# PSeitz/veloci

Measured on AMD Instinct MI355X. Metric: queries/sec, 3-term AND on 100M-doc index (p50 latency and HBM fraction alongside), higher is better.
Workload: dtype u32 doc ids + f16->f32 scores

## Files before the change

veloci_amd/csrc/capi.cpp:

```cpp
#include <chrono>
#include <thread>
#include <cstdio>
#include <cstdlib>
#include <cstring>

#include "../../include/veloci_amd.h"
#include <functional>
#include <future>

#include <dlfcn.h>
#include <unistd.h>

#include "engine.hpp"
#include "text.hpp"

using namespace vq;
using vqreq::Request;
using vqreq::VelociError;

namespace {
thread_local std::string g_err;

int fail(int code, const std::string& msg) {
    g_err = msg;
// ... 238 lines not shown
template <class F>
int debug_run(const vq_index* index, F body) {
    try {
        bool fits = true;
        vq::debug_prepass(*index->idx, [&](Workspace& ws, hipStream_t st) { fits = body(ws, st); });
        g_err.clear();
        return fits ? 0 : -2;
    } catch (const std::exception& e) {
        g_err = e.what();
        return -1;
    }
}
}

extern "C" {

const char* vq_last_error(void) { return g_err.c_str(); }
const char* vq_version(void) { return "veloci_amd 0.5 (gfx950)"; }
uint32_t vq_debug_div100_mismatches(void) { return vq::debug_div100_mismatches(); }
uint32_t vq_debug_probe_occupancy(uint32_t shape, uint32_t nd, uint32_t na, uint32_t arr_slot, uint32_t cand_cap, uint32_t* lds_bytes) {
    const size_t lds = vq::scan_probe_lds_bytes(cand_cap, nd, na, arr_slot);
    if (lds_bytes) *lds_bytes = uint32_t(lds);
    return vq::debug_probe_occupancy(shape, lds);
}
uint64_t vq_index_speculative_reruns(const vq_index* index) { return index ? index->idx->or_reruns.load() : 0; }
void vq_index_suggest_topn_probes(const vq_index* index, uint64_t* topn_probes, uint64_t* records_copied_back) {
    if (topn_probes) *topn_probes = index ? index->idx->suggest_topn_probes.load() : 0;
    if (records_copied_back) *records_copied_back = index ? index->idx->suggest_records_back.load() : 0;
}
int vq_debug_dict_topn(const uint32_t* terms, const uint32_t* classes, uint32_t n, uint32_t top_n, uint32_t* out_terms, uint32_t* out_classes, uint32_t* out_n) {
    if ((n && (!terms || !classes)) || !out_terms || !out_classes || !out_n || top_n == 0 || top_n > vq::kTopnMax) return -2;
    for (uint32_t i = 0; i < n; ++i)
        if (classes[i] >= vq::kTopnClasses) return -2;
    uint16_t ord[vq::kTopnClasses];
    vq::topn_class_ords(ord);
    return vq::debug_dict_topn(terms, classes, n, top_n, ord, out_terms, out_classes, out_n);
}
void vq_index_highlight_rank_counts(const vq_index* index, uint64_t* device_parts, uint64_t* snippets_built) {
    if (device_parts) *device_parts = index ? index->idx->highlight_device_parts.load() : 0;
    if (snippets_built) *snippets_built = index ? index->idx->highlight_snippets_built.load() : 0;
}
int vq_debug_text_rank(const uint64_t* row_off, const uint32_t* row_vals, const uint32_t* row_score_bits, uint32_t num_rows, uint32_t num_texts, uint32_t top_n,
                       uint32_t* out_texts, uint32_t* out_score_bits, uint32_t* out_n, uint32_t* out_touched) {
    if (!row_off || (num_rows && !row_score_bits) || !out_texts || !out_score_bits || !out_n || !out_touched) return -2;
    if (top_n == 0 || top_n > vq::kTextRankMaxTop || num_texts == 0 || uint64_t(num_texts) * 4 > vq::kTextRankBudget || row_off[0] != 0) return -2;
    for (uint32_t r = 0; r < num_rows; ++r) {
// ... 1389 lines not shown
```

veloci_amd/csrc/compile.cpp:

```cpp
#include <algorithm>
#include <cmath>
#include <cstdlib>
#include <cstring>
#include <regex>
#include <set>

#include "engine.hpp"
#include "text.hpp"

namespace vq {
std::atomic<uint64_t> g_compile_ns[16];

using namespace vqreq;

namespace {

bool ends_with(const std::string& s, const char* suf) {
    size_t n = std::strlen(suf);
    return s.size() >= n && std::memcmp(s.data() + s.size() - n, suf, n) == 0;
}

[[noreturn]] void unsupported(const std::string& what) {
    throw VelociError(ERR_UNSUPPORTED, "unsupported on the MI355X query path: " + what);
}
// ... 660 lines not shown
                }
                cq.algorithmic_bytes += 6ull * done->input_postings + 8ull * done->len;
                info.glen = done->global_len;
                info.len_known = !req.filtered() && idx.can_sum_over_shards();
            }
            op.list_count = uint16_t(count);
            push_op(ops, op, sp);
            info.emitted = true;
            return info;
        }
        uint32_t with_entries = 0;
        for (auto& e : entries) {
            const PostingStore& ps = *e.ps;
            if (ps.global_len[e.tid]) ++with_entries;
            if (ps.len[e.tid] == 0) continue;
            HList h;
            h.d_docs = ps.docs.as<uint32_t>() + ps.start[e.tid];
            h.d_scores = ps.scores.as<uint16_t>() + ps.start[e.tid];
            h.len = ps.len[e.tid];
            h.global_len = ps.global_len[e.tid];
            h.flags = LIST_HAS_SCORES;
            h.term_score = e.score;
            h.max_raw = ps.max_raw[e.tid];
            if (!ps.bm_start.empty() && ps.bm_start[e.tid] >= 0) {
                h.flags |= LIST_BITMAP;
                h.d_bitmap = ps.bitmaps.as<uint32_t>() + ps.bm_start[e.tid];
                h.d_rank_dir = ps.rank_dir.as<uint32_t>() + ps.rd_start[e.tid];
            }
            if (!ps.td_start.empty() && ps.td_start[e.tid] >= 0) h.d_tile_dir = ps.tile_dir.as<uint32_t>() + ps.td_start[e.tid];
            if (!ps.pk_start.empty() && ps.pk_start[e.tid] >= 0) {
                h.d_cov32 = ps.cov32.as<uint32_t>() + uint64_t(ps.pk_start[e.tid]) * 8;
                h.d_gdir = ps.gdir.as<uint32_t>() + ps.gd_start[e.tid];
                if (ps.ak_start[e.tid] >= 0) h.d_arr16 = ps.arr16.as<uint16_t>() + uint64_t(ps.ak_start[e.tid]) * 8;
                h.tile_most = ps.tile_most[e.tid];
            }
            uint32_t li = add_list(h);
            info.cover.push_back(li);
            info.cover_len += h.len;
            cq.algorithmic_bytes += 6ull * h.len;
            ++count;
        }
        op.list_count = uint16_t(count);
        info.len_known = with_entries <= 1 && !req.filtered();
        info.glen = 0;
        for (auto& e : entries) info.glen += e.ps->global_len[e.tid];
        push_op(ops, op, sp);
// ... 2132 lines not shown
```

veloci_amd/csrc/device_types.hpp:

```cpp
#pragma once
#include <hip/hip_runtime.h>
#include <stdint.h>

namespace vq {

constexpr int kBlock = 64;
constexpr int kCandCap = 2048;
constexpr int kMaxTopK = 1024;
constexpr int kStackDepth = 16;
constexpr int kMaxChildren = 16;
constexpr int kMaxLists = 64;
constexpr int kMaxOps = 160;
constexpr int kMaxSkipWhen = 4;
constexpr uint32_t kTileDirShift = 14;
constexpr uint32_t kProbeTileShift = 15;
constexpr uint32_t kRankShift = 9;

enum ListFlags : uint32_t {
    LIST_HAS_SCORES = 1u,
    LIST_COVER = 2u,
    LIST_BITMAP = 4u,
    LIST_F32 = 8u,
};

struct DList {
    const uint32_t* docs;
    const uint16_t* scores;
    uint32_t len;
    uint32_t flags;
    float term_score;
    uint16_t max_raw;
    uint16_t pad;
    const uint32_t* bitmap;
    const uint32_t* rank_dir;
    const uint32_t* tile_dir;
};

enum OpKind : uint8_t { OP_LEAF = 0, OP_AND = 1, OP_OR = 2, OP_BOOST1N = 3, OP_LEAFMAX = 4 };

struct DOp {
    uint8_t kind;
    uint8_t nchild;
    uint8_t nslots;
    uint8_t pad;
    uint16_t list_begin;
    uint16_t list_count;
    uint8_t child_slot[kMaxChildren];
    uint8_t and_order[kMaxChildren];
};

enum PresKind : uint8_t { PRES_AND = 0, PRES_OR = 1, PRES_ZERO = 2, PRES_COUNT = 3 };
constexpr uint16_t kSlotTemp = 0x8000;
constexpr uint16_t kSlotRoot = 0xFFFF;
struct DPresOp {
    uint8_t kind;
// ... 166 lines not shown
```

veloci_amd/csrc/engine.hpp:

```cpp
#pragma once
#include <hip/hip_runtime.h>

#include <atomic>
#include <cmath>
#include <chrono>
#include <cstdint>
#include <map>
#include <limits>
#include <memory>
#include <thread>
#include <functional>
#include <condition_variable>
#include <mutex>
#include <string>
#include <unordered_map>
#include <vector>

#include "device_types.hpp"
#include "kernels.hpp"
#include "request.hpp"
#include "hostpool.hpp"
#include "regex_dfa.hpp"

namespace vq {
// ... 268 lines not shown
    uint32_t len = 0;
    uint32_t total = 0;
    bool ascending = true;
    bool several = false;
    bool done = false;
};
using Boost1nTable = std::map<std::string, Boost1nJob>;
constexpr int kStatusNeedsUnion = -1;
constexpr int kStatusNeedsCounts = -2;
constexpr int kStatusNeedsRanges = -3;

struct QueryCounts {
    bool has_filter = false;
    uint64_t filter_count = 0;
    std::map<uint32_t, std::pair<uint64_t, uint64_t>> nodes;
};

struct PostingStore {
    uint32_t num_tokens = 0;
    std::vector<uint64_t> start;
    std::vector<uint32_t> len;
    std::vector<uint64_t> global_len;
    std::vector<uint16_t> max_raw;
    DevBuf docs;
    DevBuf scores;
    uint64_t total_padded = 0;
    std::vector<int64_t> bm_start;
    std::vector<int64_t> rd_start;
    DevBuf bitmaps;
    DevBuf rank_dir;
    std::vector<int64_t> td_start;
    DevBuf tile_dir;
    std::vector<int64_t> pk_start;
    std::vector<int64_t> ak_start;
    std::vector<int64_t> gd_start;
    std::vector<uint32_t> tile_most;
    DevBuf cov32, arr16, gdir;
};

struct KVStore {
    uint32_t key_base = 0, num_keys = 0;
    std::vector<uint64_t> host_off;
    std::vector<uint32_t> host_values;
    bool list_rows = false;
    bool rows_sorted_unique = true;
    bool rows_equal_postings = false;
// ... 193 lines not shown
};

std::unique_ptr<Index> build_index(const IndexBuilder& b, int device);

struct DocSet {
    uint64_t index_uid = 0;
    uint32_t num_anchors = 0, doc_lo = 0, doc_hi = 0;
    uint64_t len = 0;
    uint32_t local_len = 0;
    uint64_t bitmap_words = 0, rank_entries = 0, tile_entries = 0;
    DevBuf docs, bitmap, rank_dir, tile_dir;
    uint64_t device_bytes = 0;
    float ms_mark = -1.0f, ms_count_scan = -1.0f, ms_expand = -1.0f;
};
std::shared_ptr<const DocSet> make_docset(const Index& idx, const uint32_t* ids, uint64_t n, bool on_device);

struct HList {
    const uint32_t* d_docs = nullptr;
    const uint16_t* d_scores = nullptr;
    uint32_t len = 0;
    uint32_t flags = 0;
    float term_score = 0.f;
    uint16_t max_raw = 0x7C00;
    float max_value = std::numeric_limits<float>::infinity();
    uint64_t global_len = 0;
    const uint32_t* d_bitmap = nullptr;
    const uint32_t* d_rank_dir = nullptr;
    const uint32_t* d_tile_dir = nullptr;
    const uint32_t* d_cov32 = nullptr;
    const uint16_t* d_arr16 = nullptr;
    const uint32_t* d_gdir = nullptr;
    uint32_t tile_most = 0;
    int inline_idx = -1;
    int inline_val_idx = -1;
};

struct FacetOut {
    std::string field;
    std::string dict_path;
    uint32_t top = 10;
    uint32_t num_values = 0;
    uint32_t host_top = 0;
};

struct ExplainRec {
    enum Kind : uint8_t { Boost, MaxTokenToTextId, TermToAnchor, LevenshteinScore, OrSumOverDistinctTerms } kind = Boost;
// ... 156 lines not shown
```

veloci_amd/csrc/exec.cpp:

```cpp
#include <algorithm>
#include <cstdio>
#include <cstdlib>
#include <cstring>
#include <thread>

#include "engine.hpp"

#include "text.hpp"

namespace vq {

using namespace vqreq;

void DevBuf::ensure(size_t n) {
    if (n <= bytes) return;
    size_t want = std::max(n, bytes + bytes / 2);
    alloc(want);
}
PinnedBuf::~PinnedBuf() {
    if (p) (void)hipHostFree(p);
}
void PinnedBuf::ensure(size_t n) {
    if (n <= bytes) return;
    if (p) (void)hipHostFree(p);
// ... 121 lines not shown
    h.top_k = cq.top_k;
    h.tile_words = cq.tile_words;
    h.n_spans = cq.n_spans;
    h.keys_base = keys_base;
    h.doc_lo = idx.doc_lo;
    h.doc_hi = idx.doc_hi;
    h.part_keys_off = part_keys_off;
    h.stat_off = stat_off;
    h.blob_bytes = uint32_t(off);
    if (!dst) return off;

    std::memcpy(dst, &h, sizeof h);
    if (h.off_pool) std::memset(dst + h.off_pool, 0, sizeof(DPool) + 8 * size_t(cq.top_k));
    DList* dl = reinterpret_cast<DList*>(dst + h.off_lists);
    for (size_t i = 0; i < cq.lists.size(); ++i) {
        const HList& l = cq.lists[i];
        DList d{};
        d.docs = l.inline_idx >= 0 ? reinterpret_cast<const uint32_t*>(dev + inline_off[l.inline_idx]) : l.d_docs;
        d.scores = l.inline_val_idx >= 0 ? reinterpret_cast<const uint16_t*>(dev + inline_val_off[l.inline_val_idx]) : l.d_scores;
        d.len = l.len;
        d.flags = l.flags;
        d.term_score = l.term_score;
        d.max_raw = l.max_raw;
        d.bitmap = l.d_bitmap;
        d.rank_dir = l.d_rank_dir;
        d.tile_dir = l.d_tile_dir;
        dl[i] = d;
    }
    if (!cq.ops.empty()) std::memcpy(dst + h.off_ops, cq.ops.data(), cq.ops.size() * sizeof(DOp));
    if (!cq.fops.empty()) std::memcpy(dst + h.off_fops, cq.fops.data(), cq.fops.size() * sizeof(DOp));
    if (!cq.groups.empty()) std::memcpy(dst + h.off_groups, cq.groups.data(), cq.groups.size() * sizeof(DGroup));
    if (!cq.tboosts.empty()) std::memcpy(dst + h.off_tboost, cq.tboosts.data(), cq.tboosts.size() * sizeof(DTermBoost));
    if (!cq.cols.empty()) std::memcpy(dst + h.off_col, cq.cols.data(), cq.cols.size() * sizeof(DColBoost));
    if (!cq.locf.empty()) std::memcpy(dst + h.off_locf, cq.locf.data(), cq.locf.size() * sizeof(DLocField));
    if (!cq.loc_idx.empty()) std::memcpy(dst + h.off_loc_idx, cq.loc_idx.data(), cq.loc_idx.size() * sizeof(uint16_t));
    if (sf_rich(cq.simple_flags)) std::memcpy(dst + h.off_simple2, &cq.simple2, sizeof(DSimple2));
    if (sf_wide(cq.simple_flags)) std::memcpy(dst + h.off_simple2, &cq.wide, sizeof(DWide));
    if (sf_probe(cq.simple_flags) || sf_union_packed(cq.simple_flags)) std::memcpy(dst + h.off_simple2, &cq.probe, sizeof(DProbe));
    if (!cq.pres.empty()) std::memcpy(dst + h.off_pres, cq.pres.data(), cq.pres.size() * sizeof(DPresOp));
    if (!cq.pres_in.empty()) std::memcpy(dst + h.off_pres_in, cq.pres_in.data(), cq.pres_in.size() * sizeof(uint16_t));
    DFacet* df = reinterpret_cast<DFacet*>(dst + h.off_facets);
    for (size_t i = 0; i < cq.facets.size(); ++i) {
        DFacet f = cq.facets[i];
        f.hist_off = i < hist_off.size() ? hist_off[i] : 0u;
        f.out_off = i < fac_out_off.size() ? fac_out_off[i] : 0u;
        df[i] = f;
// ... 2431 lines not shown
```

veloci_amd/csrc/index.cpp:

```cpp
#include <algorithm>
#include <atomic>
#include <chrono>
#include <cstring>
#include <exception>
#include <mutex>
#include <thread>
#include <sys/mman.h>

#include "engine.hpp"
#include "text.hpp"

namespace vq {

const char* const TOKENS_TO_TEXT_ID = ".tokens_to_text_id";
const char* const TO_ANCHOR_ID_SCORE = ".to_anchor_id_score";
const char* const PHRASE_PAIR_TO_ANCHOR = ".phrase_pair_to_anchor";
const char* const VALUE_ID_TO_PARENT = ".value_id_to_parent";
const char* const PARENT_TO_VALUE_ID = ".parent_to_value_id";
const char* const TEXT_ID_TO_ANCHOR = ".text_id_to_anchor";
const char* const ANCHOR_TO_TEXT_ID = ".anchor_to_text_id";
const char* const BOOST_VALID_TO_VALUE = ".boost_valid_to_value";
const char* const TOKEN_VALUES = ".token_values";
const char* const VALUE_ID_TO_ANCHOR = ".value_id_to_anchor";
const char* const TEXTINDEX = ".textindex";

static bool ends_with(const std::string& s, const char* suf) {
    size_t n = std::strlen(suf);
    return s.size() >= n && std::memcmp(s.data() + s.size() - n, suf, n) == 0;
}

void DevBuf::alloc(size_t n) {
    release();
    bytes = n;
    if (n == 0) return;
    VQ_HIP(hipMalloc(&p, n));
// ... 273 lines not shown
            }
            std::vector<uint32_t> tdir(tiled.size() * (tiles + 1));
            parallel_for(tiled.size(), nthreads, [&](size_t j) {
                const uint32_t t = tiled[j];
                const uint32_t* d = docs.data() + ps.start[t];
                uint32_t* out = tdir.data() + j * (tiles + 1);
                uint32_t i = 0;
                for (uint64_t k = 0; k <= tiles; ++k) {
                    const uint64_t bound = uint64_t(idx->bitmap_base) + (k << kTileDirShift);
                    while (i < ps.len[t] && d[i] < bound) ++i;
                    out[k] = i;
                }
            });
            if (!tdir.empty()) {
                ps.tile_dir.alloc(tdir.size() * 4 + 16);
                ps.tile_dir.upload(tdir.data(), tdir.size() * 4);
                idx->device_bytes += ps.tile_dir.bytes;
            }
        }
        ps.pk_start.assign(ps.num_tokens, -1);
        ps.ak_start.assign(ps.num_tokens, -1);
        ps.gd_start.assign(ps.num_tokens, -1);
        ps.tile_most.assign(ps.num_tokens, 0);
        {
            const uint64_t ptiles = (idx->bitmap_words >> (kProbeTileShift - 5)) + 2;
            uint64_t cov_gran = 0, arr_gran = 0;
            std::vector<uint32_t> gd(tiled.size() * (ptiles + 1));
            std::vector<uint64_t> gran_of(tiled.size());
            std::vector<uint32_t> most_of(tiled.size());
            parallel_for(tiled.size(), nthreads, [&](size_t j) {
                const uint32_t t = tiled[j];
                const uint32_t* d = docs.data() + ps.start[t];
                uint32_t* g = gd.data() + j * (ptiles + 1);
                uint64_t gran = 0;
                uint32_t i = 0, most = 0;
                for (uint64_t k = 0; k <= ptiles; ++k) {
                    g[k] = uint32_t(gran);
                    const uint64_t thi = uint64_t(idx->bitmap_base) + ((k + 1) << kProbeTileShift);
                    const uint32_t i0 = i;
                    while (i < ps.len[t] && d[i] < thi) ++i;
                    const uint32_t n8 = (i - i0 + 7u) / 8u;
                    most = std::max(most, n8);
                    gran += n8;
                }
                gran_of[j] = gran;
                most_of[j] = most;
// ... 3 lines not shown
                ps.gd_start[t] = int64_t(j * (ptiles + 1));
                if (gran_of[j] >= (1ull << 28)) throw VelociError(vqreq::ERR_INVALID_ARGUMENT, "posting list too long for its tile-packed image");
                ps.pk_start[t] = int64_t(cov_gran);
                ps.tile_most[t] = most_of[j];
                cov_gran += gran_of[j];
                if (most_of[j] <= 256) {
                    ps.ak_start[t] = int64_t(arr_gran);
                    arr_gran += gran_of[j];
                }
            }
            if (cov_gran) {
                ps.cov32.alloc(cov_gran * 32 + 4096);
                ps.arr16.alloc(arr_gran * 16 + 4096);
                ps.gdir.alloc(gd.size() * 4 + 16);
                ps.gdir.upload(gd.data(), gd.size() * 4);
                idx->device_bytes += ps.cov32.bytes + ps.arr16.bytes + ps.gdir.bytes;
                uninit_vector<uint32_t> cov(cov_gran * 8);
                uninit_vector<uint16_t> arr(arr_gran * 8);
                parallel_for(tiled.size(), nthreads, [&](size_t j) {
                    const uint32_t t = tiled[j];
                    const bool as_array = ps.ak_start[t] >= 0;
                    const uint32_t* d = docs.data() + ps.start[t];
                    const uint16_t* sc = scores.data() + ps.start[t];
                    uint32_t* c = cov.data() + uint64_t(ps.pk_start[t]) * 8;
                    uint16_t* a = as_array ? arr.data() + uint64_t(ps.ak_start[t]) * 8 : nullptr;
                    uint64_t w = 0;
                    uint32_t i = 0;
                    for (uint64_t k = 0; k <= ptiles; ++k) {
                        const uint64_t tlo = uint64_t(idx->bitmap_base) + (k << kProbeTileShift), thi = tlo + (1u << kProbeTileShift);
                        for (; i < ps.len[t] && d[i] < thi; ++i, ++w) {
                            const uint32_t rel = uint32_t(d[i] - tlo);
                            c[w] = rel << 16 | sc[i];
                            if (a) a[w] = uint16_t(rel);
                        }
                        for (; w % 8; ++w) {
                            c[w] = 0xFFFFFFFFu;
                            if (a) a[w] = 0xFFFFu;
                        }
                    }
                });
                upload(ps.cov32, cov.data(), cov.size() * 4);
                upload(ps.arr16, arr.data(), arr.size() * 2);
            }
        }
        ps.docs.alloc(docs.size() * 4 + 16);
        upload(ps.docs, docs.data(), docs.size() * 4);
        ps.scores.alloc(scores.size() * 2 + 16);
        upload(ps.scores, scores.data(), scores.size() * 2);
        idx->device_bytes += ps.docs.bytes + ps.scores.bytes;
        idx->postings.emplace(path, std::move(ps));
    }

    for (auto& [path, k] : b.kv) {
        KVStore s;
        s.key_base = k.key_base;
        s.num_keys = uint32_t(k.offsets.size() - 1);
// ... 204 lines not shown
```

veloci_amd/csrc/probe_common.hpp:

```cpp
#pragma once
#include <hip/hip_runtime.h>
#include <hip/hip_fp16.h>

#include "device_types.hpp"
#include "kernel_common.hpp"

namespace vq {

__device__ __forceinline__ unsigned long long wballot(bool p) { return __builtin_amdgcn_ballot_w64(p); }

constexpr uint32_t kPT = 1u << kProbeTileShift;
constexpr uint32_t kPTW = kPT / 32;
constexpr uint32_t kPNV = kPTW / 256;
constexpr uint32_t kPRk = kPT >> kRankShift;
constexpr uint32_t kShCts = 0, kShTs = 1, kShVmax = 4, kShSrc = 7, kShPrunable = 11, kShScores = 12;

__device__ __forceinline__ void probe_lds_fence() { asm volatile("s_waitcnt lgkmcnt(0)" ::: "memory"); }

template <uint32_t ND>
struct ProbeShape {
    float cts, ts[ND], vmax[ND];
    uint32_t src[ND + 1];
    bool prunable;
};
template <uint32_t ND>
__device__ __forceinline__ ProbeShape<ND> probe_shape(const uint32_t* sh) {
    ProbeShape<ND> S;
    S.cts = __uint_as_float(sh[kShCts]);
#pragma unroll
    for (uint32_t i = 0; i < ND; ++i) {
        S.ts[i] = __uint_as_float(sh[kShTs + i]);
        S.vmax[i] = __uint_as_float(sh[kShVmax + i]);
    }
#pragma unroll
    for (uint32_t j = 0; j <= ND; ++j) S.src[j] = sh[kShSrc + j];
    S.prunable = sh[kShPrunable] != 0u;
    return S;
}
// ... 13 lines not shown
}

template <uint32_t ND>
__device__ __forceinline__ float probe_or_sum(const ProbeShape<ND>& S, float vc, const float (&vd)[ND], uint32_t mask) {
    float sum = 0.0f, nd = 0.0f;
#pragma unroll
    for (uint32_t j = 0; j <= ND; ++j) {
        float v = vc;
        bool present = true;
#pragma unroll
        for (uint32_t i = 0; i < ND; ++i)
            if (S.src[j] == 1u + i) {
                v = vd[i];
                present = ((mask >> i) & 1u) != 0u;
            }
        const float m = present ? fmaxf(0.0f, v) : 0.0f;
        if (m >= 0.00001f) nd += 1.0f;
        sum += m;
    }
    return sum * nd * nd;
}

template <uint32_t ND>
__device__ __forceinline__ uint32_t probe_raw_min(const uint32_t* sh, float thr_f, const uint32_t lane, const uint32_t or_mask = 0xFFFFFFFFu) {
    const ProbeShape<ND> S = probe_shape<ND>(sh);
    if (!S.prunable) return 0u;
    uint32_t lo = 0u, hi = 0x7C00u;
    while (hi > lo) {
        const uint32_t step = (hi - lo + 63u) >> 6;
        const uint32_t p = lo + lane * step;
        bool dead = false;
        if (p < hi) {
            const float vc = posting_value_fast(S.cts, (uint16_t)p);
            dead = (or_mask == 0xFFFFFFFFu ? probe_sum<ND>(S, vc, S.vmax) : probe_or_sum<ND>(S, vc, S.vmax, or_mask)) < thr_f;
        }
        const uint32_t c = (uint32_t)__popcll(wballot(dead));
        if (c == 0u) hi = lo;
        else {
            const uint32_t last = lo + (c - 1u) * step;
            const uint32_t nhi = last + step;
            lo = last + 1u;
            hi = nhi < hi ? nhi : hi;
        }
    }
    return lo;
}

template <bool WG>
__device__ void probe_pool_merge(const CandState& cs, uint32_t k, uint8_t* pool_bytes, const uint32_t lane) {
    uint32_t* const lock = reinterpret_cast<uint32_t*>(pool_bytes);
    uint32_t* const pn = lock + 1;
    unsigned long long* const pk = reinterpret_cast<unsigned long long*>(pool_bytes + sizeof(DPool));
    if (WG) __syncthreads();
    else probe_lds_fence();
    uint32_t n_own = *cs.n;
    n_own = n_own < cs.cap ? n_own : cs.cap;
    n_own = n_own < 32u ? n_own : 32u;
// ... 49 lines not shown
```

veloci_amd/csrc/scan_probe.hip:

```cpp
#include <hip/hip_runtime.h>
#include <hip/hip_fp16.h>

#include "device_types.hpp"
#include "kernel_common.hpp"
#include "kernels.hpp"
#include "probe_common.hpp"

namespace vq {

#ifdef VQ_STAMP
__device__ unsigned long long g_probe_stamp[16];
#define PS_INIT                                                      \
    unsigned long long _st0 = __builtin_amdgcn_s_memtime();          \
    const unsigned long long _t0 = _st0;                             \
    const unsigned long long _r0 = __builtin_amdgcn_s_memrealtime(); \
    unsigned long long _acc[16] = {0};
#define PS_AT(k)                                                \
    {                                                           \
        unsigned long long _st1 = __builtin_amdgcn_s_memtime(); \
        _acc[k] += _st1 - _st0;                                 \
        _st0 = _st1;                                            \
    }
#define PS_COUNT(k) _acc[k] += 1ull;
#define PS_FLUSH                                                                                             \
// ... 41 lines not shown
    const uint32_t sflags = H->simple_flags;
    const uint32_t top_k = H->top_k;
    constexpr uint32_t n = ND + 1u;
    constexpr uint32_t NB = ND - NA;
    constexpr uint32_t NB1 = NB ? NB : 1u, NA1 = NA ? NA : 1u;
    PS_INIT

    unsigned long long* thr = reinterpret_cast<unsigned long long*>(lds);
    uint32_t* cand_n = lds + 2;
    uint32_t* sh = lds + kPLdsShape;
    uint32_t* uq = lds + kPLdsU;
    uint32_t* rq = lds + kPLdsR;
    uint32_t* tile = lds + probe_lds_tile(ND);
    uint32_t* rank = tile + NB * kPTW;
    uint32_t* arr = lds + probe_lds_arr(ND, NB);
    unsigned long long* cand = reinterpret_cast<unsigned long long*>(arr + NA * arr_slot);
    unsigned long long* const gthr = reinterpret_cast<unsigned long long*>(const_cast<uint8_t*>(blob) + offsetof(QHeader, gthr));
    CandState cs{cand, cand_n, thr, cand_cap, gthr};
    cs.upper = H->key_upper;
    uint32_t* const stat = H->stat_off ? lds + 4 : nullptr;
    uint8_t* const pool = H->off_pool ? const_cast<uint8_t*>(blob) + H->off_pool : nullptr;

    const uint32_t* ccov = nullptr;
    const uint32_t* cgdir = nullptr;
    const uint32_t* d_bitmap[NB1];
    const uint32_t* d_rank[NB1];
    const uint16_t* d_arr[NA1];
    const uint32_t* d_agd[NA1];
    {
        const uint32_t ck = (uint32_t)__ffs((int)sf_cover_mask(sflags)) - 1u;
        const uint32_t am = sf_array_mask(sflags);
        uint32_t role_of[4] = {0u, 0u, 0u, 0u};
        uint32_t ib = 0, ia = NB;
#pragma unroll
        for (uint32_t k = 0; k < n; ++k) {
            const VQ_CONST DList& d = gl[gops[k].list_begin];
            if (k == ck) {
                ccov = P->leaf[k].cov32;
                cgdir = P->leaf[k].gdir;
                if (lane == 0) {
                    sh[kShCts] = __float_as_uint(d.term_score);
                    sh[kShPrunable] = (d.term_score > 0.0f && d.max_raw < 0x7C00u) ? 1u : 0u;
                }
            } else {
                const bool is_arr = ((am >> k) & 1u) != 0u;
                const uint32_t role = is_arr ? ia : ib;
#pragma unroll
                for (uint32_t j = 0; j < NB; ++j)
                    if (!is_arr && j == role) {
                        d_bitmap[j] = d.bitmap;
                        d_rank[j] = d.rank_dir;
                    }
#pragma unroll
                for (uint32_t a = 0; a < NA; ++a)
                    if (is_arr && NB + a == role) {
                        d_arr[a] = P->leaf[k].arr16;
                        d_agd[a] = P->leaf[k].gdir;
                    }
                if (lane == 0) {
                    const uint16_t mr = d.max_raw;
                    sh[kShTs + role] = __float_as_uint(d.term_score);
                    sh[kShVmax + role] = (d.term_score > 0.0f && mr < 0x7C00u) ? __float_as_uint(posting_value(d.term_score, mr)) : 0x7F800000u;
                    reinterpret_cast<unsigned long long*>(sh + kShScores)[role] = is_arr ? (unsigned long long)(uintptr_t)P->leaf[k].cov32 : (unsigned long long)(uintptr_t)d.scores;
                }
                role_of[k] = 1u + role;
                if (is_arr) ++ia;
                else ++ib;
            }
        }
        const KOp root(gops + n);
#pragma unroll
        for (uint32_t j = 0; j < n; ++j) {
            const uint32_t k = OR ? j : root.and_order(j);
            if (lane == 0) sh[kShSrc + j] = k == 0u ? role_of[0] : k == 1u ? role_of[1] : k == 2u ? role_of[2] : role_of[3];
        }
    }

    const uint32_t n_spans = H->n_spans;
    const unsigned long long range = (unsigned long long)(H->doc_hi - H->doc_lo);
    const uint32_t span_lo = span == 0 ? H->doc_lo : ((H->doc_lo + (uint32_t)(range * span / n_spans)) & ~(kPT - 1u));
    const uint32_t span_hi = span + 1 == n_spans ? H->doc_hi : ((H->doc_lo + (uint32_t)(range * (span + 1) / n_spans)) & ~(kPT - 1u));
    const uint32_t bitmap_base = H->bitmap_base;
    const uint32_t keys_base = H->keys_base;

    if (lane == 0) {
        *thr = __hip_atomic_load(gthr, __ATOMIC_RELAXED, __HIP_MEMORY_SCOPE_AGENT);
        *cand_n = 0;
        lds[4] = 0u;
    }
    __syncthreads();
    unsigned long long thr_seen = *thr;
    uint32_t raw_min = 0u;
    constexpr uint32_t kMasks = OR ? (1u << ND) : 1u;
    uint32_t rmin[kMasks];
    auto take_raw_min = [&](const float thr_f) {
        if (OR) {
#pragma unroll
            for (uint32_t m = 0; m < kMasks; ++m) rmin[m] = probe_raw_min<ND>(sh, thr_f, lane, m);
        } else raw_min = probe_raw_min<ND>(sh, thr_f, lane);
    };
    take_raw_min(__uint_as_float(unorder_f32((uint32_t)(thr_seen >> 32))));

    const u32x4 kSent = u32x4{0xFFFFFFFFu, 0xFFFFFFFFu, 0xFFFFFFFFu, 0xFFFFFFFFu};
    const VQ_GLOBAL u32x4* cc4 = as_global(reinterpret_cast<const u32x4*>(ccov));

    uint32_t un = 0, rn = 0;
    uint32_t ucnt = 0;
    unsigned long long hits = 0;
    unsigned long long g_prev = 0ull;

    const uint32_t t_first = (span_lo - bitmap_base) >> kProbeTileShift;
    const uint32_t t_end = span_hi > span_lo ? ((span_hi - 1u - bitmap_base) >> kProbeTileShift) + 1u : t_first;
    uint32_t dir_base = t_first;
    auto load_dir = [&](const uint32_t* g) { return as_global(g)[dir_base + lane < t_end ? dir_base + lane : t_end]; };
    uint32_t dirv = load_dir(cgdir);
    uint32_t adv[NA1];
#pragma unroll
    for (uint32_t a = 0; a < NA; ++a) adv[a] = load_dir(d_agd[a]);
    auto dir_at = [&](const uint32_t v, const uint32_t tt) { return (uint32_t)__builtin_amdgcn_readlane((int)v, (int)(tt - dir_base)); };

    u32x4 wk[ND][kPNV];
    uint32_t rk[NB1];
    u32x4 nid[kPMaxR], cid[kPMaxR];
#pragma unroll
    for (uint32_t r = 0; r < kPMaxR; ++r) nid[r] = cid[r] = kSent;
    uint32_t pf_rounds = 0, pf_v0 = 0, pf_v1 = 0;
    uint32_t na_g0[NA1], na_nv[NA1];
    uint32_t a_g0[NA1], a_cnt[NA1];
#pragma unroll
    for (uint32_t a = 0; a < NA1; ++a) na_g0[a] = na_nv[a] = a_g0[a] = a_cnt[a] = 0u;
    auto issue_tile = [&](const uint32_t tt, const uint32_t g0, const uint32_t g1) {
        pf_rounds = (g1 - g0 + 31u) >> 5;
        pf_v0 = g0 * 2u;
        pf_v1 = g1 * 2u;
        if (OR || pf_rounds) {
#pragma unroll
            for (uint32_t i = 0; i < NB; ++i) {
                const VQ_GLOBAL u32x4* gb = as_global(reinterpret_cast<const u32x4*>(d_bitmap[i] + (size_t)tt * kPTW));
#pragma unroll
                for (uint32_t h = 0; h < kPNV; ++h) wk[i][h] = gb[h * 64u + lane];
                rk[i] = as_global(d_rank[i])[tt * kPRk + lane];
// ... 56 lines not shown
    uint32_t f_mask = 0;
    auto sum_of = [&](const ProbeShape<ND>& S, const float vc, const float (&vd)[ND], const uint32_t mask) { return OR ? probe_or_sum<ND>(S, vc, vd, mask) : probe_sum<ND>(S, vc, vd); };
    auto flush_final = [&](const ProbeShape<ND>& S, const bool final) {
        const float score = sum_of(S, f_vc, f_vd, f_mask);
        const unsigned long long key = ((unsigned long long)order_f32(__float_as_uint(score)) << 32) | (unsigned long long)f_doc;
        f_stage = 0;
        PS_COUNT(12)
        push_keys(key, f_alive && key > *thr && key < cs.upper, final);
    };
    auto flush_service = [&](const bool final) {
        const unsigned long long* sptr = reinterpret_cast<const unsigned long long*>(sh + kShScores);
        unsigned long long gp = sptr[0];
        uint32_t gidx = 0u;
        if (f_stage) {
            const ProbeShape<ND> S = probe_shape<ND>(sh);
            const float thr_f = __uint_as_float(unorder_f32((uint32_t)(*thr >> 32)));
            bool last = true;
#pragma unroll
            for (uint32_t i = 0; i < ND; ++i)
                if (f_stage == i + 1u) {
                    f_vd[i] = posting_value(S.ts[i], f_r);
                    if (i + 1u < ND) {
                        constexpr uint32_t zero = 0;
                        f_alive = f_alive && !(sum_of(S, f_vc, f_vd, f_mask) < thr_f);
                        if (stat && lane == 0) *stat += 2u * (uint32_t)__popcll(wballot(f_alive));
                        gp = sptr[i + 1u < ND ? i + 1u : zero];
                        gidx = (f_alive && (!OR || ((f_mask >> (i + 1u < ND ? i + 1u : zero)) & 1u))) ? f_idx[i + 1u < ND ? i + 1u : zero] : 0u;
                        last = false;
                    }
                }
            if (last) flush_final(S, final);
            else ++f_stage;
        } else if (rn >= 64u || (final && rn)) {
            const uint32_t count = rn < 64u ? rn : 64u;
            probe_lds_fence();
            f_alive = lane < count;
            uint32_t raw = 0;
            const uint32_t slot = (rhead + lane) & (kPR - 1u);
            if (f_alive) {
                f_doc = rq[slot];
                raw = rq[kPR + slot];
#pragma unroll
                for (uint32_t i = 0; i < ND; ++i) f_idx[i] = rq[(2u + i) * kPR + slot];
            }
            if (OR) {
                f_mask = 0u;
#pragma unroll
                for (uint32_t i = 0; i < ND; ++i) f_mask |= f_idx[i] != 0xFFFFFFFFu ? 1u << i : 0u;
            }
            f_vc = posting_value(__uint_as_float(sh[kShCts]), (uint16_t)raw);
#pragma unroll
            for (uint32_t i = 0; i < ND; ++i) f_vd[i] = __uint_as_float(sh[kShVmax + i]);
            if (stat && lane == 0) *stat += 2u * count;
            gidx = (f_alive && (!OR || (f_mask & 1u))) ? f_idx[0] : 0u;
            f_stage = 1u;
            rhead = (rhead + count) & (kPR - 1u);
            rn -= count;
        }
        f_r = as_global(reinterpret_cast<const uint16_t*>((uintptr_t)gp))[gidx];
    };
    auto flush_sync = [&]() {
        const ProbeShape<ND> S = probe_shape<ND>(sh);
        probe_lds_fence();
        const uint32_t slot = (rhead + lane) & (kPR - 1u);
        const uint32_t doc = rq[slot];
        const float vc = posting_value(S.cts, (uint16_t)rq[kPR + slot]);
        float vd[ND];
        uint32_t mask = 0;
#pragma unroll
        for (uint32_t i = 0; i < ND; ++i) {
            const uint16_t* sp = reinterpret_cast<const uint16_t*>((uintptr_t) reinterpret_cast<const unsigned long long*>(sh + kShScores)[i]);
            const uint32_t ix = rq[(2u + i) * kPR + slot];
            if (ix != 0xFFFFFFFFu) mask |= 1u << i;
            vd[i] = posting_value(S.ts[i], as_global(sp)[(OR && ix == 0xFFFFFFFFu) ? 0u : ix]);
        }
        if (stat && lane == 0) *stat += 2u * ND * 64u;
        const float score = sum_of(S, vc, vd, mask);
        const unsigned long long key = ((unsigned long long)order_f32(__float_as_uint(score)) << 32) | (unsigned long long)doc;
        rhead = (rhead + 64u) & (kPR - 1u);
        rn -= 64u;
        push_keys(key, key > *thr && key < cs.upper, false);
    };
    auto bitmap_rank = [&](const uint32_t i, const uint32_t rel) {
        const uint32_t g = rel >> kRankShift, wi = (rel >> 5) & 15u, below = (1u << (rel & 31u)) - 1u;
        const int full = (int)((1u << wi) - 1u);
        const uint32_t* tl = tile + i * kPTW;
        uint32_t acc = rank[i * kPRk + g] + (uint32_t)__popc(tl[rel >> 5] & below);
        const u32x4* gw = reinterpret_cast<const u32x4*>(tl + g * 16u);
#pragma unroll
        for (uint32_t v4 = 0; v4 < 4; ++v4) {
            const u32x4 x = gw[v4];
            acc += (uint32_t)__popc(x.x & (uint32_t)__builtin_amdgcn_sbfe(full, v4 * 4u + 0u, 1u));
            acc += (uint32_t)__popc(x.y & (uint32_t)__builtin_amdgcn_sbfe(full, v4 * 4u + 1u, 1u));
            acc += (uint32_t)__popc(x.z & (uint32_t)__builtin_amdgcn_sbfe(full, v4 * 4u + 2u, 1u));
            acc += (uint32_t)__popc(x.w & (uint32_t)__builtin_amdgcn_sbfe(full, v4 * 4u + 3u, 1u));
// ... 17 lines not shown
                }
                const bool here = !OR || ((tile[role * kPTW + (rel >> 5)] >> (rel & 31u)) & 1u) != 0u;
                rq[(2u + role) * kPR + slot] = here ? bitmap_rank(role, rel) : 0xFFFFFFFFu;
            }
            rn += cnt;
        } else if (NA == 0u) {
            if (lane < cnt) {
                const uint32_t e = uqe[lane];
                const uint32_t rel = e >> 16;
                const uint32_t slot = (rhead + rn + lane) & (kPR - 1u);
                rq[slot] = tile_lo + rel;
                rq[kPR + slot] = e & 0xFFFFu;
#pragma unroll
                for (uint32_t i = 0; i < NB; ++i) {
                    const bool here = !OR || ((tile[i * kPTW + (rel >> 5)] >> (rel & 31u)) & 1u) != 0u;
                    rq[(2u + i) * kPR + slot] = here ? bitmap_rank(i, rel) : 0xFFFFFFFFu;
                }
            }
            rn += cnt;
        } else {
            uint32_t e = 0xFFFFFFFFu, pos[NA1];
            bool found = lane < cnt;
            if (found) e = uqe[lane];
            const uint32_t rel = e >> 16;
#pragma unroll
            for (uint32_t a = 0; a < NA; ++a) {
                const uint16_t* A = reinterpret_cast<const uint16_t*>(arr + a * arr_slot);
                uint32_t lo = 0u, len = a_cnt[a];
#ifdef VQ_PROBE_NO_SEARCH
                lo = rel & 7u;
                len = 0u;
#endif
                while (len > 1u) {
                    const uint32_t half = len >> 1;
                    lo = (uint32_t)A[lo + half] <= rel ? lo + half : lo;
                    len -= half;
                }
#ifdef VQ_PROBE_NO_SEARCH
                found = found && a_cnt[a] != 0u && ((uint32_t)A[lo] ^ rel) < 0x2000u;
#else
                found = found && a_cnt[a] != 0u && (uint32_t)A[lo] == rel;
#endif
                pos[a] = lo;
            }
            const unsigned long long fm = wballot(found);
            hits += (unsigned long long)__popcll(fm);
            const bool live = found && (e & 0xFFFFu) >= raw_min;
            const unsigned long long lm = wballot(live);
            if (lm) {
                if (live) {
                    const uint32_t slot = (rhead + rn + (uint32_t)__popcll(lm & ((1ull << lane) - 1ull))) & (kPR - 1u);
                    rq[slot] = tile_lo + rel;
                    rq[kPR + slot] = e & 0xFFFFu;
#pragma unroll
                    for (uint32_t i = 0; i < NB; ++i) rq[(2u + i) * kPR + slot] = bitmap_rank(i, rel);
#pragma unroll
                    for (uint32_t a = 0; a < NA; ++a) rq[(2u + NB + a) * kPR + slot] = (a_g0[a] * 8u + pos[a]) * 2u;
                }
                rn += (uint32_t)__popcll(lm);
            }
        }
    };
    uint32_t lo_rel = 0, width = 0;
    struct ProbeWords {
        uint32_t w[OR ? ND : 1u][4];
    };
    auto probe_read = [&](const u32x4 e4) {
        const uint32_t ee[4] = {e4.x, e4.y, e4.z, e4.w};
        ProbeWords pw;
#pragma unroll
        for (uint32_t c = 0; c < 4; ++c) {
            const uint32_t a = (ee[c] >> 21) & (kPTW - 1u);
            if (OR) {
#pragma unroll
                for (uint32_t i = 0; i < ND; ++i) pw.w[OR ? i : 0u][c] = tile[i * kPTW + a];
            } else {
                pw.w[0][c] = 0xFFFFFFFFu;
                if (NB) {
                    pw.w[0][c] = tile[a];
#pragma unroll
// ... 6 lines not shown
    auto probe_eval = [&](const u32x4 e4, const ProbeWords& pw, const bool may_overflow) {
        const uint32_t ee[4] = {e4.x, e4.y, e4.z, e4.w};
        unsigned long long lm[4];
        bool live[4];
#pragma unroll
        for (uint32_t c = 0; c < 4; ++c) {
            const uint32_t rel = ee[c] >> 16;
            const bool in = (rel - lo_rel) < width;
            if (OR) {
                uint32_t mask = 0;
#pragma unroll
                for (uint32_t i = 0; i < ND; ++i) mask |= ((pw.w[OR ? i : 0u][c] >> (rel & 31u)) & 1u) << i;
                uint32_t need = rmin[0];
#pragma unroll
                for (uint32_t m = 1; m < kMasks; ++m) need = mask == m ? rmin[OR ? m : 0u] : need;
                hits += (unsigned long long)__popcll(wballot(in && mask == 0u));
                live[c] = in && (ee[c] & 0xFFFFu) >= need;
                lm[c] = wballot(live[c]);
                continue;
            }
            const bool bit = ((pw.w[0][c] >> (rel & 31u)) & 1u) != 0u;
            const unsigned long long sm = NB ? (wballot(in) & wballot(bit)) : wballot(in);
            if (NA == 0u) {
                const bool strong = (ee[c] & 0xFFFFu) >= raw_min;
                hits += (unsigned long long)__popcll(sm);
                lm[c] = sm & wballot(strong);
                live[c] = in && bit && strong;
            } else {
                lm[c] = sm;
                live[c] = in && bit;
            }
        }
        if (lm[0] | lm[1] | lm[2] | lm[3]) {
            if (may_overflow) {
                const uint32_t add = (uint32_t)__popcll(lm[0]) + (uint32_t)__popcll(lm[1]) + (uint32_t)__popcll(lm[2]) + (uint32_t)__popcll(lm[3]);
                while (un + add > kPU) rank_some(un < 64u ? un : 64u);
            }
#pragma unroll
            for (uint32_t c = 0; c < 4; ++c) {
                if (live[c]) uq[un + (uint32_t)__popcll(lm[c] & ((1ull << lane) - 1ull))] = ee[c];
                un += (uint32_t)__popcll(lm[c]);
            }
        }
    };

    uint32_t t = t_first;
    tile_lo = bitmap_base + (t_first << kProbeTileShift);
// ... 39 lines not shown
                a_cnt[a] = na_nv[a] * 8u;
            }
#pragma unroll
            for (uint32_t r = 0; r < kPMaxR; ++r) {
                cid[r] = nid[r];
                asm volatile("" : "+v"(cid[r]));
            }
        }
        {
            uint32_t fr = f_r, glo = (uint32_t)g_prev, ghi = (uint32_t)(g_prev >> 32);
            asm volatile("" : "+v"(fr), "+v"(glo), "+v"(ghi), "+v"(dirv));
#pragma unroll
            for (uint32_t a = 0; a < NA; ++a) asm volatile("" : "+v"(adv[a]));
            f_r = (uint16_t)fr;
            g_prev = ((unsigned long long)ghi << 32) | glo;
        }
        PS_AT(1)
        if (lane == 0 && g_prev > *thr) *thr = g_prev;
        const bool more = t + 1u < t_end;
        uint32_t ng0 = 0, ng1 = 0;
        if (more) {
            if (t + 2u - dir_base >= 64u) {
                dir_base = t + 1u;
                dirv = load_dir(cgdir);
#pragma unroll
                for (uint32_t a = 0; a < NA; ++a) adv[a] = load_dir(d_agd[a]);
            }
            ng0 = dir_at(dirv, t + 1u);
            ng1 = dir_at(dirv, t + 2u);
            next_arrays(t + 1u);
        }
        if (f_stage || rn >= 64u) PS_COUNT(11)
        flush_service(false);
        PS_AT(4)
        if (more) issue_tile(t + 1u, ng0, ng1);
        else pf_rounds = 0;
        if (lane == 0) g_prev = __hip_atomic_load(gthr, __ATOMIC_RELAXED, __HIP_MEMORY_SCOPE_AGENT);
        __builtin_amdgcn_s_setprio(0);
        probe_lds_fence();
        {
            const unsigned long long tn = *thr;
            if ((uint32_t)(tn >> 32) != (uint32_t)(thr_seen >> 32)) take_raw_min(__uint_as_float(unorder_f32((uint32_t)(tn >> 32))));
            thr_seen = tn;
            ++tiles_since_merge;
        }
        PS_AT(5)
#ifdef VQ_PROBE_STREAM_ONLY
        hits += (unsigned long long)__popcll(wballot((cid[0].x ^ cid[1].y) == 0x12345u));
        if (rounds && span == 0xFFFFFFFFu) {
// ... 145 lines not shown
```

Measured before the change: 163,200.

## Tag low-score array postings with class bit for tighter per-class pruning bounds

At index build, each arr16 entry now packs a 15-bit in-tile offset plus a class bit marking postings whose score is at or below a per-term pivot. The pivot is chosen so roughly one eighth of postings lie above it. In the AND probe kernel, a separate raw-score minimum is computed for each combination of array-term classes, using the lower pivot value as that term's bound. Candidates that matched only low-class array entries can then be rejected earlier, saving scoring work and random score fetches. The cost is extra LDS slots and readfirstlane'd thresholds, a wider binary-search key encoding, and recomputing gdir pointers from the blob instead of holding them in registers, which may raise per-tile overhead.

```diff
diff --git a/veloci_amd/csrc/capi.cpp b/veloci_amd/csrc/capi.cpp
--- a/veloci_amd/csrc/capi.cpp
+++ b/veloci_amd/csrc/capi.cpp
@@ -284,6 +284,21 @@
     const size_t lds = vq::scan_probe_lds_bytes(cand_cap, nd, na, arr_slot);
     if (lds_bytes) *lds_bytes = uint32_t(lds);
     return vq::debug_probe_occupancy(shape, lds);
+}
+uint64_t vq_debug_arr16_list(const vq_index* index, const char* store_path, uint32_t token, uint16_t* out, uint64_t cap, uint16_t* pivot_raw, uint16_t* max_raw) {
+    if (!index || !store_path) return 0;
+    auto it = index->idx->postings.find(store_path);
+    if (it == index->idx->postings.end()) return 0;
+    const PostingStore& ps = it->second;
+    if (token >= ps.num_tokens || ps.ak_start.empty() || ps.ak_start[token] < 0) return 0;
+    const uint64_t ptiles = (index->idx->bitmap_words >> (kProbeTileShift - 5)) + 2;
+    uint32_t gran = 0;
+    if (hipMemcpy(&gran, ps.gdir.as<uint32_t>() + ps.gd_start[token] + ptiles, 4, hipMemcpyDeviceToHost) != hipSuccess) return 0;
+    const uint64_t n = uint64_t(gran) * 8, take = std::min(n, cap);
+    if (take && out && hipMemcpy(out, ps.arr16.as<uint16_t>() + uint64_t(ps.ak_start[token]) * 8, take * 2, hipMemcpyDeviceToHost) != hipSuccess) return 0;
+    if (pivot_raw) *pivot_raw = ps.pivot_raw[token];
+    if (max_raw) *max_raw = ps.max_raw[token];
+    return n;
 }
 uint64_t vq_index_speculative_reruns(const vq_index* index) { return index ? index->idx->or_reruns.load() : 0; }
 void vq_index_suggest_topn_probes(const vq_index* index, uint64_t* topn_probes, uint64_t* records_copied_back) {
diff --git a/veloci_amd/csrc/compile.cpp b/veloci_amd/csrc/compile.cpp
--- a/veloci_amd/csrc/compile.cpp
+++ b/veloci_amd/csrc/compile.cpp
@@ -706,6 +706,7 @@
             h.flags = LIST_HAS_SCORES;
             h.term_score = e.score;
             h.max_raw = ps.max_raw[e.tid];
+            h.pivot_raw = ps.pivot_raw[e.tid];
             if (!ps.bm_start.empty() && ps.bm_start[e.tid] >= 0) {
                 h.flags |= LIST_BITMAP;
                 h.d_bitmap = ps.bitmaps.as<uint32_t>() + ps.bm_start[e.tid];
diff --git a/veloci_amd/csrc/device_types.hpp b/veloci_amd/csrc/device_types.hpp
--- a/veloci_amd/csrc/device_types.hpp
+++ b/veloci_amd/csrc/device_types.hpp
@@ -14,6 +14,12 @@
 constexpr int kMaxSkipWhen = 4;
 constexpr uint32_t kTileDirShift = 14;
 constexpr uint32_t kProbeTileShift = 15;
+static_assert(kProbeTileShift == 15, "an arr16 entry holds a 15-bit in-tile offset and a class bit");
+constexpr uint32_t kArrPadRel = (1u << kProbeTileShift) - 1u;
+#ifndef VQ_SCORE_CLASS_DIV
+#define VQ_SCORE_CLASS_DIV 8
+#endif
+constexpr uint32_t kScoreClassDiv = VQ_SCORE_CLASS_DIV;
 constexpr uint32_t kRankShift = 9;
 
 enum ListFlags : uint32_t {
@@ -30,7 +36,7 @@
     uint32_t flags;
     float term_score;
     uint16_t max_raw;
-    uint16_t pad;
+    uint16_t pivot_raw;
     const uint32_t* bitmap;
     const uint32_t* rank_dir;
     const uint32_t* tile_dir;
diff --git a/veloci_amd/csrc/engine.hpp b/veloci_amd/csrc/engine.hpp
--- a/veloci_amd/csrc/engine.hpp
+++ b/veloci_amd/csrc/engine.hpp
@@ -314,6 +314,7 @@
     std::vector<uint32_t> len;
     std::vector<uint64_t> global_len;
     std::vector<uint16_t> max_raw;
+    std::vector<uint16_t> pivot_raw;
     DevBuf docs;
     DevBuf scores;
     uint64_t total_padded = 0;
@@ -553,6 +554,7 @@
     uint32_t flags = 0;
     float term_score = 0.f;
     uint16_t max_raw = 0x7C00;
+    uint16_t pivot_raw = 0x7C00;
     float max_value = std::numeric_limits<float>::infinity();
     uint64_t global_len = 0;
     const uint32_t* d_bitmap = nullptr;
diff --git a/veloci_amd/csrc/exec.cpp b/veloci_amd/csrc/exec.cpp
--- a/veloci_amd/csrc/exec.cpp
+++ b/veloci_amd/csrc/exec.cpp
@@ -167,6 +167,7 @@
         d.flags = l.flags;
         d.term_score = l.term_score;
         d.max_raw = l.max_raw;
+        d.pivot_raw = l.pivot_raw;
         d.bitmap = l.d_bitmap;
         d.rank_dir = l.d_rank_dir;
         d.tile_dir = l.d_tile_dir;
diff --git a/veloci_amd/csrc/index.cpp b/veloci_amd/csrc/index.cpp
--- a/veloci_amd/csrc/index.cpp
+++ b/veloci_amd/csrc/index.cpp
@@ -11,6 +11,19 @@
 #include "text.hpp"
 
 namespace vq {
+
+uint16_t score_class_pivot(const uint16_t* sc, uint32_t len, uint16_t max_raw) {
+    if (len == 0 || max_raw >= 0x7C00u) return max_raw;
+    std::vector<uint32_t> count(size_t(max_raw) + 1, 0u);
+    for (uint32_t i = 0; i < len; ++i) ++count[sc[i]];
+    const uint64_t need = (uint64_t(len) + kScoreClassDiv - 1) / kScoreClassDiv;
+    uint64_t above = 0;
+    for (uint32_t r = max_raw; r-- > 0;) {
+        above += count[r + 1];
+        if (above >= need && count[r]) return uint16_t(r);
+    }
+    return max_raw;
+}
 
 const char* const TOKENS_TO_TEXT_ID = ".tokens_to_text_id";
 const char* const TO_ANCHOR_ID_SCORE = ".to_anchor_id_score";
@@ -330,6 +343,7 @@
         ps.ak_start.assign(ps.num_tokens, -1);
         ps.gd_start.assign(ps.num_tokens, -1);
         ps.tile_most.assign(ps.num_tokens, 0);
+        ps.pivot_raw = ps.max_raw;
         {
             const uint64_t ptiles = (idx->bitmap_words >> (kProbeTileShift - 5)) + 2;
             uint64_t cov_gran = 0, arr_gran = 0;
@@ -379,6 +393,9 @@
                     const bool as_array = ps.ak_start[t] >= 0;
                     const uint32_t* d = docs.data() + ps.start[t];
                     const uint16_t* sc = scores.data() + ps.start[t];
+                    if (as_array) ps.pivot_raw[t] = score_class_pivot(sc, ps.len[t], ps.max_raw[t]);
+                    const uint16_t pivot = ps.pivot_raw[t];
+                    const bool classed = as_array && pivot < ps.max_raw[t];
                     uint32_t* c = cov.data() + uint64_t(ps.pk_start[t]) * 8;
                     uint16_t* a = as_array ? arr.data() + uint64_t(ps.ak_start[t]) * 8 : nullptr;
                     uint64_t w = 0;
@@ -388,7 +405,7 @@
                         for (; i < ps.len[t] && d[i] < thi; ++i, ++w) {
                             const uint32_t rel = uint32_t(d[i] - tlo);
                             c[w] = rel << 16 | sc[i];
-                            if (a) a[w] = uint16_t(rel);
+                            if (a) a[w] = uint16_t(rel << 1 | ((classed && sc[i] <= pivot && rel != kArrPadRel) ? 1u : 0u));
                         }
                         for (; w % 8; ++w) {
                             c[w] = 0xFFFFFFFFu;
diff --git a/veloci_amd/csrc/probe_common.hpp b/veloci_amd/csrc/probe_common.hpp
--- a/veloci_amd/csrc/probe_common.hpp
+++ b/veloci_amd/csrc/probe_common.hpp
@@ -13,7 +13,7 @@
 constexpr uint32_t kPTW = kPT / 32;
 constexpr uint32_t kPNV = kPTW / 256;
 constexpr uint32_t kPRk = kPT >> kRankShift;
-constexpr uint32_t kShCts = 0, kShTs = 1, kShVmax = 4, kShSrc = 7, kShPrunable = 11, kShScores = 12;
+constexpr uint32_t kShCts = 0, kShTs = 1, kShVmax = 4, kShSrc = 7, kShPrunable = 11, kShScores = 12, kShVlow = 18;
 
 __device__ __forceinline__ void probe_lds_fence() { asm volatile("s_waitcnt lgkmcnt(0)" ::: "memory"); }
 
@@ -73,9 +73,12 @@
 }
 
 template <uint32_t ND>
-__device__ __forceinline__ uint32_t probe_raw_min(const uint32_t* sh, float thr_f, const uint32_t lane, const uint32_t or_mask = 0xFFFFFFFFu) {
+__device__ __forceinline__ uint32_t probe_raw_min(const uint32_t* sh, float thr_f, const uint32_t lane, const uint32_t or_mask = 0xFFFFFFFFu, const uint32_t low_mask = 0u) {
     const ProbeShape<ND> S = probe_shape<ND>(sh);
     if (!S.prunable) return 0u;
+    float vb[ND];
+#pragma unroll
+    for (uint32_t i = 0; i < ND; ++i) vb[i] = ((low_mask >> i) & 1u) ? __uint_as_float(sh[kShVlow + i]) : S.vmax[i];
     uint32_t lo = 0u, hi = 0x7C00u;
     while (hi > lo) {
         const uint32_t step = (hi - lo + 63u) >> 6;
@@ -83,7 +86,7 @@
         bool dead = false;
         if (p < hi) {
             const float vc = posting_value_fast(S.cts, (uint16_t)p);
-            dead = (or_mask == 0xFFFFFFFFu ? probe_sum<ND>(S, vc, S.vmax) : probe_or_sum<ND>(S, vc, S.vmax, or_mask)) < thr_f;
+            dead = (or_mask == 0xFFFFFFFFu ? probe_sum<ND>(S, vc, vb) : probe_or_sum<ND>(S, vc, vb, or_mask)) < thr_f;
         }
         const uint32_t c = (uint32_t)__popcll(wballot(dead));
         if (c == 0u) hi = lo;
diff --git a/veloci_amd/csrc/scan_probe.hip b/veloci_amd/csrc/scan_probe.hip
--- a/veloci_amd/csrc/scan_probe.hip
+++ b/veloci_amd/csrc/scan_probe.hip
@@ -87,11 +87,9 @@
     uint8_t* const pool = H->off_pool ? const_cast<uint8_t*>(blob) + H->off_pool : nullptr;
 
     const uint32_t* ccov = nullptr;
-    const uint32_t* cgdir = nullptr;
     const uint32_t* d_bitmap[NB1];
     const uint32_t* d_rank[NB1];
     const uint16_t* d_arr[NA1];
-    const uint32_t* d_agd[NA1];
     {
         const uint32_t ck = (uint32_t)__ffs((int)sf_cover_mask(sflags)) - 1u;
         const uint32_t am = sf_array_mask(sflags);
@@ -102,7 +100,6 @@
             const VQ_CONST DList& d = gl[gops[k].list_begin];
             if (k == ck) {
                 ccov = P->leaf[k].cov32;
-                cgdir = P->leaf[k].gdir;
                 if (lane == 0) {
                     sh[kShCts] = __float_as_uint(d.term_score);
                     sh[kShPrunable] = (d.term_score > 0.0f && d.max_raw < 0x7C00u) ? 1u : 0u;
@@ -118,14 +115,14 @@
                     }
 #pragma unroll
                 for (uint32_t a = 0; a < NA; ++a)
-                    if (is_arr && NB + a == role) {
-                        d_arr[a] = P->leaf[k].arr16;
-                        d_agd[a] = P->leaf[k].gdir;
-                    }
+                    if (is_arr && NB + a == role) d_arr[a] = P->leaf[k].arr16;
                 if (lane == 0) {
                     const uint16_t mr = d.max_raw;
                     sh[kShTs + role] = __float_as_uint(d.term_score);
-                    sh[kShVmax + role] = (d.term_score > 0.0f && mr < 0x7C00u) ? __float_as_uint(posting_value(d.term_score, mr)) : 0x7F800000u;
+                    const bool bounded = d.term_score > 0.0f && mr < 0x7C00u;
+                    const uint32_t vmax_bits = bounded ? __float_as_uint(posting_value(d.term_score, mr)) : 0x7F800000u;
+                    sh[kShVmax + role] = vmax_bits;
+                    sh[kShVlow + role] = (bounded && is_arr && d.pivot_raw < mr) ? __float_as_uint(posting_value(d.term_score, d.pivot_raw)) : vmax_bits;
                     reinterpret_cast<unsigned long long*>(sh + kShScores)[role] = is_arr ? (unsigned long long)(uintptr_t)P->leaf[k].cov32 : (unsigned long long)(uintptr_t)d.scores;
                 }
                 role_of[k] = 1u + role;
@@ -155,14 +152,15 @@
     }
     __syncthreads();
     unsigned long long thr_seen = *thr;
-    uint32_t raw_min = 0u;
-    constexpr uint32_t kMasks = OR ? (1u << ND) : 1u;
+    constexpr uint32_t kMasks = OR ? (1u << ND) : (1u << NA);
     uint32_t rmin[kMasks];
     auto take_raw_min = [&](const float thr_f) {
-        if (OR) {
-#pragma unroll
-            for (uint32_t m = 0; m < kMasks; ++m) rmin[m] = probe_raw_min<ND>(sh, thr_f, lane, m);
-        } else raw_min = probe_raw_min<ND>(sh, thr_f, lane);
+#pragma unroll
+        for (uint32_t m = 0; m < kMasks; ++m) {
+            const uint32_t r = OR ? probe_raw_min<ND>(sh, thr_f, lane, m) : probe_raw_min<ND>(sh, thr_f, lane, 0xFFFFFFFFu, m << NB);
+            if (!OR && NA) probe_lds_fence();
+            rmin[m] = (!OR && NA) ? (uint32_t)__builtin_amdgcn_readfirstlane((int)r) : r;
+        }
     };
     take_raw_min(__uint_as_float(unorder_f32((uint32_t)(thr_seen >> 32))));
 
@@ -177,11 +175,24 @@
     const uint32_t t_first = (span_lo - bitmap_base) >> kProbeTileShift;
     const uint32_t t_end = span_hi > span_lo ? ((span_hi - 1u - bitmap_base) >> kProbeTileShift) + 1u : t_first;
     uint32_t dir_base = t_first;
-    auto load_dir = [&](const uint32_t* g) { return as_global(g)[dir_base + lane < t_end ? dir_base + lane : t_end]; };
-    uint32_t dirv = load_dir(cgdir);
+    auto load_dir = [&](const uint32_t which) {
+        const uint8_t* b = blob;
+        asm volatile("" : "+s"(b));
+        const VQ_CONST QHeader* Hb = as_const<QHeader>(b);
+        const uint32_t sf = Hb->simple_flags;
+        uint32_t k = (uint32_t)__ffs((int)sf_cover_mask(sf)) - 1u;
+        if (which) {
+            uint32_t am = sf_array_mask(sf);
+            for (uint32_t a = 1; a < which; ++a) am &= am - 1u;
+            k = (uint32_t)__ffs((int)am) - 1u;
+        }
+        const uint32_t* g = as_const<DProbe>(b + Hb->off_simple2)->leaf[k].gdir;
+        return as_global(g)[dir_base + lane < t_end ? dir_base + lane : t_end];
+    };
+    uint32_t dirv = load_dir(0u);
     uint32_t adv[NA1];
 #pragma unroll
-    for (uint32_t a = 0; a < NA; ++a) adv[a] = load_dir(d_agd[a]);
+    for (uint32_t a = 0; a < NA; ++a) adv[a] = load_dir(1u + a);
     auto dir_at = [&](const uint32_t v, const uint32_t tt) { return (uint32_t)__builtin_amdgcn_readlane((int)v, (int)(tt - dir_base)); };
 
     u32x4 wk[ND][kPNV];
@@ -284,10 +295,14 @@
                     f_vd[i] = posting_value(S.ts[i], f_r);
                     if (i + 1u < ND) {
                         constexpr uint32_t zero = 0;
-                        f_alive = f_alive && !(sum_of(S, f_vc, f_vd, f_mask) < thr_f);
+                        const uint32_t nx = i + 1u < ND ? i + 1u : zero;
+                        float vb[ND];
+#pragma unroll
+                        for (uint32_t j = 0; j < ND; ++j) vb[j] = (j > i && j >= NB && (f_idx[j] & 1u)) ? __uint_as_float(sh[kShVlow + j]) : f_vd[j];
+                        f_alive = f_alive && !(sum_of(S, f_vc, vb, f_mask) < thr_f);
                         if (stat && lane == 0) *stat += 2u * (uint32_t)__popcll(wballot(f_alive));
-                        gp = sptr[i + 1u < ND ? i + 1u : zero];
-                        gidx = (f_alive && (!OR || ((f_mask >> (i + 1u < ND ? i + 1u : zero)) & 1u))) ? f_idx[i + 1u < ND ? i + 1u : zero] : 0u;
+                        gp = sptr[nx];
+                        gidx = (f_alive && (!OR || ((f_mask >> nx) & 1u))) ? (nx >= NB ? f_idx[nx] & ~1u : f_idx[nx]) : 0u;
                         last = false;
                     }
                 }
@@ -314,7 +329,7 @@
 #pragma unroll
             for (uint32_t i = 0; i < ND; ++i) f_vd[i] = __uint_as_float(sh[kShVmax + i]);
             if (stat && lane == 0) *stat += 2u * count;
-            gidx = (f_alive && (!OR || (f_mask & 1u))) ? f_idx[0] : 0u;
+            gidx = (f_alive && (!OR || (f_mask & 1u))) ? (NB ? f_idx[0] : f_idx[0] & ~1u) : 0u;
             f_stage = 1u;
             rhead = (rhead + count) & (kPR - 1u);
             rn -= count;
@@ -332,7 +347,8 @@
 #pragma unroll
         for (uint32_t i = 0; i < ND; ++i) {
             const uint16_t* sp = reinterpret_cast<const uint16_t*>((uintptr_t) reinterpret_cast<const unsigned long long*>(sh + kShScores)[i]);
-            const uint32_t ix = rq[(2u + i) * kPR + slot];
+            uint32_t ix = rq[(2u + i) * kPR + slot];
+            if (!OR && i >= NB) ix &= ~1u;
             if (ix != 0xFFFFFFFFu) mask |= 1u << i;
             vd[i] = posting_value(S.ts[i], as_global(sp)[(OR && ix == 0xFFFFFFFFu) ? 0u : ix]);
         }
@@ -396,40 +412,52 @@
             uint32_t e = 0xFFFFFFFFu, pos[NA1];
             bool found = lane < cnt;
             if (found) e = uqe[lane];
-            const uint32_t rel = e >> 16;
+            {
+                const uint32_t off = e >> 16;
+                e = (off * 2u + 1u < 0xFFFEu ? off * 2u + 1u : 0xFFFEu) << 16 | (e & 0xFFFFu);
+                asm volatile("" : "+v"(e));
+            }
 #pragma unroll
             for (uint32_t a = 0; a < NA; ++a) {
                 const uint16_t* A = reinterpret_cast<const uint16_t*>(arr + a * arr_slot);
                 uint32_t lo = 0u, len = a_cnt[a];
 #ifdef VQ_PROBE_NO_SEARCH
-                lo = rel & 7u;
+                lo = (e >> 17) & 7u;
                 len = 0u;
 #endif
                 while (len > 1u) {
                     const uint32_t half = len >> 1;
-                    lo = (uint32_t)A[lo + half] <= rel ? lo + half : lo;
+                    lo = (uint32_t)A[lo + half] <= (e >> 16) ? lo + half : lo;
                     len -= half;
                 }
 #ifdef VQ_PROBE_NO_SEARCH
-                found = found && a_cnt[a] != 0u && ((uint32_t)A[lo] ^ rel) < 0x2000u;
+                const uint32_t ent = A[lo];
+                found = found && a_cnt[a] != 0u && ((ent >> 1) ^ (e >> 17)) < 0x2000u;
 #else
-                found = found && a_cnt[a] != 0u && (uint32_t)A[lo] == rel;
+                const uint32_t ent = A[lo];
+                found = found && a_cnt[a] != 0u && (ent >> 1) == (e >> 17);
 #endif
-                pos[a] = lo;
+                pos[a] = lo * 2u | (ent & 1u);
             }
             const unsigned long long fm = wballot(found);
             hits += (unsigned long long)__popcll(fm);
-            const bool live = found && (e & 0xFFFFu) >= raw_min;
+            uint32_t cls = 0u;
+#pragma unroll
+            for (uint32_t a = 0; a < NA; ++a) cls |= (pos[a] & 1u) << a;
+            bool live = found && (e & 0xFFFFu) >= rmin[0];
+#pragma unroll
+            for (uint32_t m = 1; m < kMasks; ++m) live = live && !(cls == m && (e & 0xFFFFu) < rmin[(!OR && NA) ? m : 0u]);
             const unsigned long long lm = wballot(live);
             if (lm) {
                 if (live) {
+                    const uint32_t rel = e >> 17;
                     const uint32_t slot = (rhead + rn + (uint32_t)__popcll(lm & ((1ull << lane) - 1ull))) & (kPR - 1u);
                     rq[slot] = tile_lo + rel;
                     rq[kPR + slot] = e & 0xFFFFu;
 #pragma unroll
                     for (uint32_t i = 0; i < NB; ++i) rq[(2u + i) * kPR + slot] = bitmap_rank(i, rel);
 #pragma unroll
-                    for (uint32_t a = 0; a < NA; ++a) rq[(2u + NB + a) * kPR + slot] = (a_g0[a] * 8u + pos[a]) * 2u;
+                    for (uint32_t a = 0; a < NA; ++a) rq[(2u + NB + a) * kPR + slot] = a_g0[a] * 16u + pos[a];
                 }
                 rn += (uint32_t)__popcll(lm);
             }
@@ -482,7 +510,7 @@
             const bool bit = ((pw.w[0][c] >> (rel & 31u)) & 1u) != 0u;
             const unsigned long long sm = NB ? (wballot(in) & wballot(bit)) : wballot(in);
             if (NA == 0u) {
-                const bool strong = (ee[c] & 0xFFFFu) >= raw_min;
+                const bool strong = (ee[c] & 0xFFFFu) >= rmin[0];
                 hits += (unsigned long long)__popcll(sm);
                 lm[c] = sm & wballot(strong);
                 live[c] = in && bit && strong;
@@ -568,9 +596,9 @@
         if (more) {
             if (t + 2u - dir_base >= 64u) {
                 dir_base = t + 1u;
-                dirv = load_dir(cgdir);
-#pragma unroll
-                for (uint32_t a = 0; a < NA; ++a) adv[a] = load_dir(d_agd[a]);
+                dirv = load_dir(0u);
+#pragma unroll
+                for (uint32_t a = 0; a < NA; ++a) adv[a] = load_dir(1u + a);
             }
             ng0 = dir_at(dirv, t + 1u);
             ng1 = dir_at(dirv, t + 2u);
```

New measurement: 177,300, median of 6. 8.6% higher.
